# cheukwaylee/ORB_SLAM2_detailed_comments

Hardware: AMD Instinct MI355X
Metric: frames/sec ORB extract+match (1000 kp, 640x480) (higher is better)
Workload: dtype u8; 1 GPU; synthetic 640x480 mono stream, nFeatures=1000, 8 levels, scale 1.2, FAST 20/7, extract+match(t vs t-1), batch 1024 frames/GPU resident in HBM, 1 pipelines/GPU; parallelism=single GPU

## Files before the change

### include/orbx.h

```cpp
#ifndef ORBX_H
#define ORBX_H
#include <stddef.h>
#include <stdint.h>
#ifdef __cplusplus
extern "C" {
#endif

#define ORBX_ABI_VERSION 1

typedef struct orbx_keypoint {
    float x, y;
    float size;
    float angle;
    float response;
    int32_t octave;
    int32_t class_id;
} orbx_keypoint;

typedef enum orbx_status {
    ORBX_OK = 0,
    ORBX_EMPTY_IMAGE = 1,
    ORBX_BAD_ARGUMENT = 2,
    ORBX_BAD_ASPECT = 3,
    ORBX_CAPACITY = 4,
// ... 336 lines not shown
void *orbx_get_stream(orbx_handle *h);
orbx_status orbx_set_stream(orbx_handle *h, void *hip_stream);
orbx_status orbx_synchronize(orbx_handle *h);
enum {
    ORBX_K_PYR_L0 = 0, ORBX_K_PYR_RESIZE = 1, ORBX_K_FAST = 2, ORBX_K_QUADTREE = 3, ORBX_K_ORIENT = 4,
    ORBX_K_BLUR = 5, ORBX_K_DESC = 6, ORBX_K_MATCH = 7, ORBX_K_MISC = 8, ORBX_K_COUNT = 9
};
orbx_status orbx_profile_enable(orbx_handle *h, uint32_t kernel_mask);
orbx_status orbx_profile_read(orbx_handle *h, float *ms, int32_t *launches, int reset);
const char *orbx_kernel_name(int kernel_id);

orbx_status orbx_debug_candidates(orbx_handle *h, int frame, int level, orbx_keypoint *out, int cap, int *n);
orbx_status orbx_debug_level_keypoints(orbx_handle *h, int frame, int level, orbx_keypoint *out, int cap, int *n);
orbx_status orbx_debug_blur_copy(orbx_handle *h, int frame, int level, uint8_t *dst, int dst_stride);
orbx_status orbx_debug_fast_groups(orbx_handle *h, int *level0, int *total);

typedef struct orbx_pose_problem {
    int32_t frame;
    float   Tcw[16];
    const int32_t *point_index;
    int32_t npoints;
} orbx_pose_problem;
orbx_status orbx_pose_optimization_batch_device(orbx_handle *h, int nproblems, const orbx_pose_problem *problems, int npool,
                                                const float *world_pos, int nframes, const orbx_keypoint *d_keys_un,
                                                const float *d_u_right, const int32_t *d_counts, int cap, const int32_t *d_point,
                                                const float *camera4, float mbf, const float *inv_level_sigma2, int nlevels,
                                                float *d_Tcw, uint8_t *d_outlier, int32_t *d_ninliers);
orbx_status orbx_pose_optimization(orbx_handle *h, float *Tcw, int n, const orbx_keypoint *keys_un, const float *u_right,
                                   const int32_t *point, int npool, const float *world_pos, const float *camera4, float mbf,
                                   const float *inv_level_sigma2, int nlevels, uint8_t *outlier, int32_t *ninliers);
// ... 31 lines not shown
```

### orb_slam2_detailed_comments_amd/_capi.py

```python
from __future__ import annotations
import ctypes as C
import os
import numpy as np

HERE = os.path.dirname(os.path.abspath(__file__))
LIB_PATH = os.environ.get("ORBX_LIB") or os.path.join(HERE, "lib", "liborbx.so")

KP_DTYPE = np.dtype([("x", "<f4"), ("y", "<f4"), ("size", "<f4"), ("angle", "<f4"),
                     ("response", "<f4"), ("octave", "<i4"), ("class_id", "<i4")])
assert KP_DTYPE.itemsize == 28

OK, EMPTY_IMAGE, BAD_ARGUMENT, BAD_ASPECT, CAPACITY, HIP_ERROR, NO_DEVICE, UNSUPPORTED = range(8)
FP_GCC_FMA, FP_STRICT = 0, 1
PYRAMID_FORK_PADDED, PYRAMID_UPSTREAM = 0, 1
FMT_GRAY8, FMT_RGB8, FMT_BGR8, FMT_RGBA8, FMT_BGRA8 = range(5)
DEPTH_U16, DEPTH_F32 = 0, 1
K_NAMES = ("k_pyr_l0", "k_pyr_resize", "k_fast_rows", "k_quadtree", "k_orient", "k_blur", "k_describe",
           "k_match", "misc")
K_COUNT = len(K_NAMES)


class Params(C.Structure):
    _fields_ = [("nfeatures", C.c_int32), ("scale_factor", C.c_float), ("nlevels", C.c_int32),
                ("ini_th_fast", C.c_int32), ("min_th_fast", C.c_int32), ("pyramid_mode", C.c_int32),
# ... 82 lines not shown

class OrbxError(RuntimeError):
    def __init__(self, status, msg):
        super().__init__(f"orbx status {status}: {msg}")
        self.status = status


SYMBOLS = [
    "orbx_create", "orbx_destroy", "orbx_default_params", "orbx_last_error", "orbx_status_string",
    "orbx_abi_version", "orbx_get_levels", "orbx_get_scale_factor", "orbx_get_scale_tables",
    "orbx_get_features_per_level", "orbx_get_umax", "orbx_max_keypoints", "orbx_extract", "orbx_extract_batch",
    "orbx_extract_batch_device", "orbx_pyramid_level_info", "orbx_pyramid_level_device",
    "orbx_pyramid_level_copy", "orbx_match_bruteforce_device", "orbx_match_bruteforce", "orbx_hamming_matrix",
    "orbx_get_stream", "orbx_set_stream", "orbx_synchronize", "orbx_profile_enable", "orbx_profile_read",
    "orbx_kernel_name", "orbx_debug_candidates", "orbx_debug_level_keypoints", "orbx_debug_blur_copy", "orbx_debug_fast_groups",
    "orbx_grid_create", "orbx_grid_destroy", "orbx_grid_query", "orbx_three_maxima",
    "orbx_search_for_initialization", "orbx_stereo_match", "orbx_search_by_projection_frame",
    "orbx_search_by_projection_mappoints", "orbx_search_by_projection_frame_batch_device",
    "orbx_search_by_projection_mappoints_batch_device", "orbx_predict_scale_table", "orbx_predict_scale",
    "orbx_search_local_points_batch_device", "orbx_set_input_format", "orbx_search_by_bow_keyframe_frame",
    "orbx_search_by_bow_keyframes", "orbx_search_by_bow_keyframe_frame_batch", "orbx_search_by_bow_keyframes_batch", "orbx_search_for_triangulation", "orbx_triangulation_batch_create", "orbx_triangulation_batch_select", "orbx_triangulation_batch_destroy", "orbx_fuse", "orbx_fuse_sim3", "orbx_fuse_batch", "orbx_fuse_sim3_batch",
    "orbx_search_by_projection_sim3", "orbx_search_by_sim3", "orbx_search_by_projection_keyframe",
    "orbx_stereo_match_batch_device", "orbx_host_alloc", "orbx_host_free", "orbx_set_rectification", "orbx_undistort_keypoints_device",
    "orbx_grid_build_device", "orbx_gated_candidates",
    "orbx_undistort_keypoints", "orbx_image_bounds", "orbx_rgbd_depth_device", "orbx_rgbd_depth", "orbx_extract_rgbd_batch",
    "orbx_vocabulary_create", "orbx_vocabulary_destroy", "orbx_bow_transform", "orbx_bow_transform_device", "orbx_bow_vectors",
    "orbx_vocabulary_scoring", "orbx_bow_score", "orbx_kfdb_create", "orbx_kfdb_destroy", "orbx_kfdb_clear", "orbx_kfdb_size",
    "orbx_kfdb_add", "orbx_kfdb_erase", "orbx_kfdb_score_entries", "orbx_kfdb_query_reloc", "orbx_kfdb_query_loop",
    "orbx_kfdb_query_matches", "orbx_kfdb_query_touched", "orbx_kfdb_select_groups", "orbx_kfdb_state",
    "orbx_distinctive_descriptors_batch", "orbx_distinctive_descriptors_batch_device", "orbx_update_normal_and_depth_batch",
# ... 62 lines not shown
    L.orbx_sim3_batch_counts.restype = i32; L.orbx_sim3_batch_counts.argtypes = [vp, i32, vp, C.POINTER(i32)]
    L.orbx_sim3_batch_hypothesis.restype = i32; L.orbx_sim3_batch_hypothesis.argtypes = [vp, i32, i32, vp, vp]
    L.orbx_sim3_batch_destroy.restype = None; L.orbx_sim3_batch_destroy.argtypes = [vp]
    L.orbx_sim3_atan2.restype = C.c_double; L.orbx_sim3_atan2.argtypes = [C.c_double, C.c_double]
    L.orbx_get_stream.restype = vp; L.orbx_get_stream.argtypes = [vp]
    L.orbx_set_stream.restype = i32; L.orbx_set_stream.argtypes = [vp, vp]
    L.orbx_synchronize.restype = i32; L.orbx_synchronize.argtypes = [vp]
    L.orbx_profile_enable.restype = i32; L.orbx_profile_enable.argtypes = [vp, C.c_uint32]
    L.orbx_profile_read.restype = i32; L.orbx_profile_read.argtypes = [vp, vp, vp, i32]
    L.orbx_kernel_name.restype = C.c_char_p; L.orbx_kernel_name.argtypes = [i32]
    L.orbx_debug_candidates.restype = i32; L.orbx_debug_candidates.argtypes = [vp, i32, i32, vp, i32, C.POINTER(i32)]
    L.orbx_debug_level_keypoints.restype = i32
    L.orbx_debug_level_keypoints.argtypes = [vp, i32, i32, vp, i32, C.POINTER(i32)]
    L.orbx_debug_blur_copy.restype = i32; L.orbx_debug_blur_copy.argtypes = [vp, i32, i32, vp, i32]
    L.orbx_debug_fast_groups.restype = i32; L.orbx_debug_fast_groups.argtypes = [vp, C.POINTER(i32), C.POINTER(i32)]
    L.orbx_grid_create.restype = vp; L.orbx_grid_create.argtypes = [vp, i32, f32, f32, f32, f32]
    L.orbx_grid_destroy.restype = None; L.orbx_grid_destroy.argtypes = [vp]
    L.orbx_grid_query.restype = i32; L.orbx_grid_query.argtypes = [vp, f32, f32, f32, i32, i32, vp, i32]
    L.orbx_three_maxima.restype = None
    L.orbx_three_maxima.argtypes = [vp, i32, C.POINTER(i32), C.POINTER(i32), C.POINTER(i32)]
    L.orbx_search_for_initialization.restype = i32
    L.orbx_search_for_initialization.argtypes = [vp, vp, vp, i32, vp, vp, i32, vp, vp, i32, f32, i32, vp, C.POINTER(i32)]
    L.orbx_stereo_match.restype = i32
    L.orbx_stereo_match.argtypes = [vp, vp, i32, i32, vp, vp, i32, vp, vp, i32, f32, f32, vp, vp, C.POINTER(i32)]
    L.orbx_search_by_projection_frame.restype = i32
    L.orbx_search_by_projection_frame.argtypes = [vp, C.POINTER(FrameView), C.POINTER(LastFrameView), f32, i32, i32, vp,
                                                  C.POINTER(i32)]
    L.orbx_search_by_projection_mappoints.restype = i32
    L.orbx_search_by_projection_mappoints.argtypes = [vp, C.POINTER(FrameView), vp, C.POINTER(MapPointView), f32, f32, vp,
                                                      C.POINTER(i32)]
# ... 120 lines not shown
```

### orb_slam2_detailed_comments_amd/csrc/orbx_kernels.hip

```cpp
#include "orbx_device.h"
#include "orbx_inplace.h"
#include "orbx_fast_net.h"
#include "orbx_track.h"
#include "../../include/orbx_pattern_data.h"

#define L0_ROWS 8
#ifndef L0_FF
#define L0_FF 1
#endif
#ifndef RR_FF
#define RR_FF 1
#endif
#define QT_KPT ORBX_QT_KPT
#ifndef QT_DROP_STAGE_A
#define QT_DROP_STAGE_A 1
#endif
#ifndef QT_ONE_SCAN
#define QT_ONE_SCAN 1
#endif
#ifndef QT_REG_SIZE
#define QT_REG_SIZE 1
#endif
#ifndef QT_CENSUS_NODES
#define QT_CENSUS_NODES 1
// ... 1543 lines not shown
                s0 = s0 + (float)r3 * k3;
                o = (int)__builtin_rintf(s0);
            } else {
                o = (55 * r0 + 49 * r1 + 34 * r2 + 18 * r3 + (1 << 15)) >> 16;
            }
            o = min(max(o, 0), 255);
            outv |= (uint32_t)o << (8 * i);
        }
        *(uint32_t *)(out + (long long)Y * L.pitch + X) = outv;
    }
}

__constant__ int4 c_pattern_lane[64];
__constant__ uint32_t c_orient_w[64][12];
__constant__ uint32_t c_blur_b[3][64][4];

#ifndef DS_ORDER
#define DS_ORDER 1
#endif
#define DS_R 21
#define DS_W (2 * DS_R + 1)
#define DS_PP 44
#define DS_HC 40
#ifndef DS_COLFIRST
#define DS_COLFIRST 1
#endif
#ifndef DS_ALIAS
#define DS_ALIAS 1
#endif
#ifndef DS_MFMA
#define DS_MFMA 1
#endif
#define DS_VC 44
#define DS_VR 40
#ifndef DS_WPB
#define DS_WPB 1
#endif
#ifndef DS_WPS
#define DS_WPS 7
#endif
typedef const __attribute__((address_space(3))) uint16_t *orbx_lds_u16p;
typedef const __attribute__((address_space(3))) uint32_t *orbx_lds_u32p;
__device__ __forceinline__ uint32_t orbx_ds_tap(uint32_t adr) {
    typedef unsigned short u16x2 __attribute__((ext_vector_type(2)));
    const bool odd = (adr & 2u) != 0;
    const orbx_lds_u32p wp = (orbx_lds_u32p)(uintptr_t)(adr & ~3u);
    const uint32_t d0 = wp[0], d1 = wp[1], d2 = wp[2], d3 = wp[3];
    const uint32_t w0 = odd ? (18u << 16) : (18u | (34u << 16)), w1 = odd ? (34u | (49u << 16)) : (49u | (55u << 16)),
                   w2 = odd ? (55u | (49u << 16)) : (49u | (34u << 16)), w3 = odd ? (34u | (18u << 16)) : 18u;
    uint32_t I = __builtin_amdgcn_udot2(__builtin_bit_cast(u16x2, d0), __builtin_bit_cast(u16x2, w0), 0u, false);
    I = __builtin_amdgcn_udot2(__builtin_bit_cast(u16x2, d1), __builtin_bit_cast(u16x2, w1), I, false);
    I = __builtin_amdgcn_udot2(__builtin_bit_cast(u16x2, d2), __builtin_bit_cast(u16x2, w2), I, false);
    I = __builtin_amdgcn_udot2(__builtin_bit_cast(u16x2, d3), __builtin_bit_cast(u16x2, w3), I, false);
    return I;
}
template <int FPM, bool INPLACE>
__global__ __launch_bounds__(64 * DS_WPB, DS_WPS) void k_describe(DGeom g, const uint8_t *__restrict__ pyr,
                                                  const uint32_t *__restrict__ lvl_kp,
                                                  const int *__restrict__ lvl_count,
                                                  float *__restrict__ lvl_angle, orbx_keypoint *__restrict__ kps,
                                                  uint8_t *__restrict__ desc, int *__restrict__ counts,
                                                  int *__restrict__ status, int cap, int dbg_stop, int nframes, OrbxRaw0 raw) {
#ifndef ORBX_TIMING_KNOBS
    dbg_stop = 0;
#endif
#if DS_COLFIRST && DS_ALIAS
    __shared__ __attribute__((aligned(16))) uint16_t s_h[DS_WPB][DS_VR * DS_VC];
#else
    __shared__ uint32_t s_patch[DS_WPB][DS_W * DS_PP / 4 + 4];
    __shared__ __attribute__((aligned(16))) uint16_t s_h[DS_WPB][DS_COLFIRST ? DS_VR * DS_VC : DS_W * DS_HC];
#endif
    const int lane = threadIdx.x & 63, wv_id = __builtin_amdgcn_readfirstlane(threadIdx.x >> 6);
#if DS_ORDER == 1
    const int f = blockIdx.y * 8 + (blockIdx.x & 7);
    const int oi = (blockIdx.x >> 3) * DS_WPB + wv_id;
    if (f >= nframes) return;
#else
    const int f = blockIdx.x;
    const int oi = blockIdx.y * DS_WPB + wv_id;
#endif
    const int *lc = lvl_count + f * g.nlevels;
    int total = 0, level = 0, slot = oi;
#ifndef DS_LEVELS8
#define DS_LEVELS8 1
#endif
    if (DS_LEVELS8 && g.nlevels == 8) {
        const int4 ca = *(const int4 *)lc, cb = *(const int4 *)(lc + 4);
        const int cnt[8] = {ca.x, ca.y, ca.z, ca.w, cb.x, cb.y, cb.z, cb.w};
        int base = 0;
#pragma unroll
        for (int l = 0; l < 8; ++l) {
            if (oi >= total) { level = l; base = total; }
            total += cnt[l];
        }
        slot = g.lv[level].kp_begin + (oi - base);
    } else {
#pragma unroll
    for (int l = 0; l < ORBX_MAX_LEVELS; ++l) {
        if (l < g.nlevels) {
            if (oi >= total) { level = l; slot = g.lv[l].kp_begin + (oi - total); }
            total += lc[l];
        }
    }
    }
    if (oi == 0 && lane == 0) {
        counts[f] = min(total, cap);
        if (total > cap) atomicMax(&status[f], (int)ORBX_CAPACITY);
    }
    if (oi >= min(total, cap) || dbg_stop == 4) return;
#if DS_COLFIRST && DS_ALIAS
    uint32_t *patch = (uint32_t *)s_h[wv_id];
#else
    uint32_t *patch = s_patch[wv_id];
#endif
    uint16_t *hrow = s_h[wv_id];
    const uint32_t pos = lvl_kp[(long long)f * g.kp_total + slot];
    const int4 pat = c_pattern_lane[lane];
    const DLevel &L = g.lv[level];
    const int x = (int)(pos & 0xfff) + (ORBX_EDGE - 3), y = (int)((pos >> 12) & 0xfff) + (ORBX_EDGE - 3);
    const bool ip0 = INPLACE && level == 0;
    const uint8_t *img = ip0 ? raw.img + (long long)f * raw.frame_stride : pyr + (long long)f * g.pyr_bytes + L.off;
    const int spitch = ip0 ? raw.stride : L.pitch;
    const int px0 = x - DS_R + (ip0 ? -ORBX_EDGE : L.org), py0 = y - DS_R + (ip0 ? -ORBX_EDGE : L.org);
    const int xa = px0 & ~3;
    const bool interior = ip0 ? orbx_ip_desc_interior(px0, py0, raw.W, raw.H)
                              : px0 >= 0 && py0 >= 0 && xa + 48 <= L.pitch && px0 + 2 * DS_R < L.pw && py0 + 2 * DS_R < L.ph;
    {
        if (interior) {
            const int dq = lane & 3, rq = lane >> 2;
            const uint32_t shift = (uint32_t)(px0 & 3);
            const uint8_t *p0 = img + (__mul24(py0, spitch) + xa + 12 * dq);
            orbx_uint3_u tv[3];
#pragma unroll
            for (int k = 0; k < 3; ++k) tv[k] = *(const orbx_uint3_u *)(p0 + __mul24(min(16 * k + rq, DS_W - 1), spitch));
#pragma unroll
            for (int k = 0; k < 3; ++k) {
                const uint32_t nxt = orbx_lane_above(tv[k].x);
                const int r = 16 * k + rq;
                if (r < DS_W) {
                    uint32_t *d = patch + r * (DS_PP / 4) + 3 * dq;
                    d[0] = __builtin_amdgcn_alignbyte(tv[k].y, tv[k].x, shift);
                    d[1] = __builtin_amdgcn_alignbyte(tv[k].z, tv[k].y, shift);
                    if (dq < 3) d[2] = __builtin_amdgcn_alignbyte(nxt, tv[k].z, shift);
                }
            }
        } else if (ip0) {
            const int dq = lane & 3, rq = lane >> 2;
            const int ws = orbx_ip_desc_ws(px0, raw.W);
            const int e = px0 - ws;
            const uint32_t shift = (uint32_t)(e & 3);
            const int dd = e >> 2;
            orbx_uint3_u tv[3];
#pragma unroll
            for (int k = 0; k < 3; ++k)
                tv[k] = *(const orbx_uint3_u *)(img + orbx_ip_row_off(orbx_ip_map(py0 + ORBX_EDGE + min(16 * k + rq, DS_W - 1), raw.H), raw.stride, ws + 12 * dq));
#pragma unroll
            for (int k = 0; k < 3; ++k) {
                const uint32_t nxt = orbx_lane_above(tv[k].x);
                const int r = 16 * k + rq;
                if (r < DS_W) {
                    uint32_t *d = patch + r * (DS_PP / 4);
                    const int D = 3 * dq - dd;
                    const uint32_t f0 = __builtin_amdgcn_alignbyte(tv[k].y, tv[k].x, shift), f1 = __builtin_amdgcn_alignbyte(tv[k].z, tv[k].y, shift),
                                   f2 = __builtin_amdgcn_alignbyte(nxt, tv[k].z, shift);
                    if (D >= 0 && D < DS_PP / 4) d[D] = f0;
                    if (D + 1 >= 0 && D + 1 < DS_PP / 4) d[D + 1] = f1;
                    if (D + 2 >= 0 && D + 2 < DS_PP / 4) d[D + 2] = f2;
                    if (dq == 0 && D - 1 >= 0 && D - 1 < DS_PP / 4) d[D - 1] = __builtin_amdgcn_alignbyte(tv[k].x, 0u, shift);
                }
            }
            const int c_end_l = px0 < 0 ? min(-px0, DS_W) : 0, c_beg_r = max(raw.W - px0, 0);
            if (c_end_l > 0 || c_beg_r < DS_W) {
                orbx_wave_sync();
                uint8_t *pb = (uint8_t *)patch + min(lane, DS_W - 1) * DS_PP;
                const uint8_t *grow = img + orbx_ip_row_off(orbx_ip_map(py0 + ORBX_EDGE + min(lane, DS_W - 1), raw.H), raw.stride, 0);
                for (int c = 0; c < DS_W; ++c) {
                    if (c >= c_end_l && c < c_beg_r) { c = c_beg_r - 1; continue; }
                    const int j = orbx_ip_map(px0 + ORBX_EDGE + c, raw.W);
                    const int sp = j - px0;
                    const uint8_t v = (sp >= 0 && sp < DS_PP) ? pb[sp] : grow[j];
                    if (lane < DS_W) pb[c] = v;
                }
            }
        } else {
            uint8_t *pb = (uint8_t *)patch;
            for (int i = lane; i < DS_W * DS_W; i += 64) {
                const int r = i / DS_W, c = i - r * DS_W;
                const int sy = orbx_reflect101(py0 + r, L.ph), sx = orbx_reflect101(px0 + c, L.pw);
                pb[r * DS_PP + c] = img[(long long)sy * L.pitch + sx];
            }
        }
        orbx_wave_sync();
        if (dbg_stop == 1) return;
        float angle_deg;
        {
            const int row = lane >> 1, half = lane & 1;
            const uint32_t *pr = patch + min(row + (DS_R - ORBX_HALF_PATCH), DS_W - 1) * (DS_PP / 4) + 1 + 5 * half;
            const uint4 wa = *(const uint4 *)&c_orient_w[lane][0], wb = *(const uint4 *)&c_orient_w[lane][4], wc = *(const uint4 *)&c_orient_w[lane][8];
            const uint32_t p0 = pr[0], p1 = pr[1], p2 = pr[2], p3 = pr[3], p4 = pr[4];
            uint32_t A = __builtin_amdgcn_udot4(p0, wa.x, 0u, false), S = __builtin_amdgcn_udot4(p0, wb.y, 0u, false);
            A = __builtin_amdgcn_udot4(p1, wa.y, A, false); S = __builtin_amdgcn_udot4(p1, wb.z, S, false);
            A = __builtin_amdgcn_udot4(p2, wa.z, A, false); S = __builtin_amdgcn_udot4(p2, wb.w, S, false);
            A = __builtin_amdgcn_udot4(p3, wa.w, A, false); S = __builtin_amdgcn_udot4(p3, wc.x, S, false);
            A = __builtin_amdgcn_udot4(p4, wb.x, A, false); S = __builtin_amdgcn_udot4(p4, wc.y, S, false);
            int m10 = (int)A - 16 * (int)S;
            int m01 = __mul24(row - ORBX_HALF_PATCH, (int)S);
            m10 = orbx_wave_sum(m10);
            m01 = orbx_wave_sum(m01);
            angle_deg = orbx_fast_atan2((float)m01, (float)m10);
            if (lane == 0) lvl_angle[(long long)f * g.kp_total + slot] = angle_deg;
        }
        if (dbg_stop == 2) return;
#if DS_COLFIRST && DS_MFMA
        {
            typedef int i32x4 __attribute__((ext_vector_type(4)));
            const int m = lane & 15, gq = lane >> 4;
            i32x4 A[3], Bm[3];
#pragma unroll
            for (int t = 0; t < 3; ++t) {
                const uint32_t *ap = patch + (16 * t + m) * (DS_PP / 4) + 4 * gq;
                A[t][0] = (int)(ap[0] ^ 0x80808080u); A[t][1] = (int)(ap[1] ^ 0x80808080u);
                A[t][2] = (int)(ap[2] ^ 0x80808080u); A[t][3] = (int)(ap[3] ^ 0x80808080u);
            }
#pragma unroll
            for (int j = 0; j < 3; ++j) {
                const uint4 b4 = *(const uint4 *)&c_blur_b[j][lane][0];
                Bm[j][0] = (int)b4.x; Bm[j][1] = (int)b4.y; Bm[j][2] = (int)b4.z; Bm[j][3] = (int)b4.w;
            }
            const i32x4 c0 = {128 * 257, 128 * 257, 128 * 257, 128 * 257};
            uint32_t *vo = (uint32_t *)hrow + m * (DS_VC / 2) + 2 * gq;
#pragma unroll
            for (int j = 0; j < 3; ++j) {
#pragma unroll
                for (int t = 0; t < 3; ++t) {
                    const i32x4 acc = __builtin_amdgcn_mfma_i32_16x16x64_i8(A[t], Bm[j], c0, 0, 0, 0);
                    if ((j < 2 || m < DS_W - 6 - 32) && (t < 2 || gq < 3))
                        *(uint2 *)(vo + (16 * j) * (DS_VC / 2) + 8 * t) =
                            make_uint2((uint32_t)acc[0] | ((uint32_t)acc[1] << 16), (uint32_t)acc[2] | ((uint32_t)acc[3] << 16));
                }
            }
        }
#elif DS_COLFIRST
        {
            typedef unsigned short u16x2 __attribute__((ext_vector_type(2)));
            const int seg = (lane * 373) >> 12, cg = lane - 11 * seg;
            if (seg < 5) {
                uint32_t pa[14], pb[14];
#pragma unroll
                for (int j = 0; j < 14; ++j) {
                    const uint32_t d = patch[min(8 * seg + j, DS_W - 1) * (DS_PP / 4) + cg];
                    pa[j] = __builtin_amdgcn_perm(0u, d, 0x0c010c00u);
                    pb[j] = __builtin_amdgcn_perm(0u, d, 0x0c030c02u);
                }
// ... 29 lines not shown
            o.y = hv[2] | (hv[3] << 16);
            o.z = hv[4] | (hv[5] << 16);
            o.w = hv[6] | (hv[7] << 16);
            *(uint4 *)(hrow + r * DS_HC + 8 * q8) = o;
        }
#endif
        __builtin_amdgcn_fence(__ATOMIC_RELEASE, "wavefront");
        __builtin_amdgcn_wave_barrier();
        __builtin_amdgcn_fence(__ATOMIC_ACQUIRE, "wavefront");
        if (dbg_stop == 3) return;
        const float factorPI = (float)(3.1415926535897932384626433832795 / 180.f);
        const float angle = angle_deg * factorPI;
                const OrbxSinCos sc = orbx_sincosf_pinned(angle);
        const float a = sc.c, b = sc.s;
        const int wvec = (L.pw - 2 * L.org) & ~3;
        const int pw4[4] = {pat.x, pat.y, pat.z, pat.w};
        unsigned long long words[4];
        if (x + (DS_R - 3) < wvec) {
#if DS_COLFIRST
            const uint32_t cbias = (uint32_t)(2 * ((DS_R - 3) * DS_VC + (DS_R - 3))) - 0x400000u * (2u * DS_VC) - (0x4B400000u << 1);
#else
            const uint32_t cbias = (uint32_t)(2 * ((DS_R - 3) * DS_HC + (DS_R - 3))) - 0x400000u * (2u * DS_HC) - (0x4B400000u << 1);
#endif
            const uint32_t hbase = (uint32_t)(uintptr_t)(orbx_lds_u16p)hrow + cbias;
            float tv[8];
            float nb = -b;
            asm("" : "+v"(nb));
#pragma unroll
            for (int r = 0; r < 4; ++r) {
#pragma unroll
                for (int s2 = 0; s2 < 2; ++s2) {
                    const float px = (float)(signed char)((pw4[r] >> (16 * s2)) & 0xff);
                    const float py = (float)(signed char)((pw4[r] >> (16 * s2 + 8)) & 0xff);
                    float fy, fx;
                    if (FPM == ORBX_FP_GCC_FMA) {
                        fy = __builtin_fmaf(px, b, py * a);
                        fx = __builtin_fmaf(px, a, py * nb);
                    } else {
                        fy = px * b + py * a;
                        fx = px * a + py * nb;
                    }
                    const uint32_t uy = __float_as_uint(fy + 12582912.0f), ux = __float_as_uint(fx + 12582912.0f);
#if DS_COLFIRST
#if DS_MFMA
                    uint32_t ay = (uy << 1) + hbase;
                    asm("" : "+v"(ay));
                    const uint32_t adr = __umul24(ux, 2u * DS_VC) + ay;
#else
                    const uint32_t adr = __umul24(uy, 2u * DS_VC) + ((ux << 1) + hbase);
#endif
                    const uint32_t I = orbx_ds_tap(adr);
#else
                    uint32_t adr = __umul24(uy, 2u * DS_HC) + ((ux << 1) + hbase);
                    asm("" : "+v"(adr));
                    const orbx_lds_u16p hp = (orbx_lds_u16p)(uintptr_t)adr;
                    const uint32_t r0 = hp[3 * DS_HC], r1 = (uint32_t)hp[2 * DS_HC] + hp[4 * DS_HC],
                                   r2 = (uint32_t)hp[1 * DS_HC] + hp[5 * DS_HC], r3 = (uint32_t)hp[0] + hp[6 * DS_HC];
                    const uint32_t I = __umul24(55u, r0) + __umul24(49u, r1) + __umul24(34u, r2) + __umul24(18u, r3);
#endif
                    tv[2 * r + s2] = __builtin_fminf(__builtin_rintf((float)I * (1.f / 65536.f)), 255.f);
                }
            }
#pragma unroll
            for (int r = 0; r < 4; ++r) words[r] = orbx_ballot(tv[2 * r] < tv[2 * r + 1]);
        } else {
            int tval[8];
#pragma unroll
            for (int r = 0; r < 4; ++r) {
#pragma unroll
                for (int s2 = 0; s2 < 2; ++s2) {
                    const float px = (float)(signed char)((pw4[r] >> (16 * s2)) & 0xff);
                    const float py = (float)(signed char)((pw4[r] >> (16 * s2 + 8)) & 0xff);
                    float fy, fx;
                    if (FPM == ORBX_FP_GCC_FMA) {
                        fy = __builtin_fmaf(px, b, py * a);
                        fx = __builtin_fmaf(px, a, -(py * b));
                    } else {
                        fy = px * b + py * a;
                        fx = px * a - py * b;
                    }
                    const int iy = (int)__builtin_rintf(fy), ix = (int)__builtin_rintf(fx);
#if DS_COLFIRST
#if DS_MFMA
                    const uint32_t I = orbx_ds_tap((uint32_t)(uintptr_t)(orbx_lds_u16p)hrow + 2u * (uint32_t)(__mul24(ix + DS_R - 3, DS_VC) + (iy + DS_R - 3)));
#else
                    const uint32_t I = orbx_ds_tap((uint32_t)(uintptr_t)(orbx_lds_u16p)hrow + 2u * (uint32_t)(__mul24(iy + DS_R - 3, DS_VC) + (ix + DS_R - 3)));
#endif
#else
                    const uint16_t *hp = hrow + __mul24(iy + DS_R - 3, DS_HC) + (ix + DS_R - 3);
                    const uint32_t r0 = hp[3 * DS_HC], r1 = (uint32_t)hp[2 * DS_HC] + hp[4 * DS_HC],
                                   r2 = (uint32_t)hp[1 * DS_HC] + hp[5 * DS_HC], r3 = (uint32_t)hp[0] + hp[6 * DS_HC];
                    const uint32_t I = __umul24(55u, r0) + __umul24(49u, r1) + __umul24(34u, r2) + __umul24(18u, r3);
#endif
                    const uint32_t tie = x + ix >= wvec ? 1u : ((I >> 16) & 1u);
                    tval[2 * r + s2] = (int)min((I + 0x7fffu + tie) >> 16, 255u);
                }
            }
#pragma unroll
            for (int r = 0; r < 4; ++r) words[r] = orbx_ballot(tval[2 * r] < tval[2 * r + 1]);
        }
        if (lane < 4) {
            unsigned long long w = lane == 0 ? words[0] : lane == 1 ? words[1] : lane == 2 ? words[2] : words[3];
            *(unsigned long long *)(desc + ((long long)f * cap + oi) * 32 + 8 * lane) = w;
        }
        if (lane == 0) {
            orbx_keypoint kp;
            float fx = (float)x, fy = (float)y;
            if (level != 0) { fx = fx * L.scale; fy = fy * L.scale; }
            kp.x = fx; kp.y = fy;
            kp.size = L.size;
// ... 1835 lines not shown
            const bool in = i < len && orbx_sim3_inlier(T12, T21, K1, K2, v, v + 3, v + 8, v + 10, v[6], v[7]);
            const unsigned long long word = orbx_ballot(in);
            if (lane == 0) mw[(base + sub) >> 6] = word;
            cnt += __popcll(word);
        }
    }
    if (active && lane == 0) A.counts[D.iter_off + it] = cnt;
}

#include "orbx_launch.h"
#include <string>
#include <cstdio>
#include <cstring>
#include <mutex>

hipError_t orbx_upload_pattern() {
    signed char t[64 * 16];
    for (int l = 0; l < 64; ++l)
        for (int r = 0; r < 4; ++r)
            for (int k = 0; k < 4; ++k) t[l * 16 + r * 4 + k] = ORBX_PATTERN_I8[(r * 64 + l) * 4 + k];
    hipError_t e = hipMemcpyToSymbol(HIP_SYMBOL(c_pattern_lane), t, sizeof(t));
    if (e != hipSuccess) return e;
    orbx_params p;
    orbx_default_params(&p);
    OrbxTables tab;
    orbx_build_tables(p, tab);
    static uint32_t w[64][12];
    memset(w, 0, sizeof(w));
    for (int lane = 0; lane < 62; ++lane) {
        const int row = lane >> 1, half = lane & 1, v = row - ORBX_HALF_PATCH;
        const int d = tab.umax[v < 0 ? -v : v];
        for (int k = 0; k < 5; ++k)
            for (int b = 0; b < 4; ++b) {
                const int col = 4 * (1 + 5 * half + k) + b;
                const int u = col - DS_R;
                if (col < DS_W && u >= -d && u <= d) {
// ... 384 lines not shown
```

### orb_slam2_detailed_comments_amd/csrc/orbx_launch.h

```cpp
#pragma once
#include <hip/hip_runtime.h>
#include "orbx_device.h"
#include "orbx_inplace.h"
#include "orbx_track.h"
#include "orbx_mappoint.h"
#include "orbx_pose.h"
#include "orbx_sim3.h"

hipError_t orbx_upload_pattern();
size_t orbx_quadtree_smem(int ncap, int lds_keys);
hipError_t orbx_quadtree_prepare(size_t smem);
void orbx_launch_clear(hipStream_t s, int *a, int na, int *b, int nb, int *c, int nc);
void orbx_launch_pyr_l0(hipStream_t s, const DGeom &g, int B, const uint8_t *imgs, int W, int H, int stride,
                        long long frame_stride, uint8_t *pyr, int *status, int *cand_cursor);
void orbx_launch_pyr_l0_color(hipStream_t s, const DGeom &g, int B, const uint8_t *imgs, int W, int H, int stride,
                              long long frame_stride, uint8_t *pyr, int nch, int r_off, int b_off, int *status, int *cand_cursor);
void orbx_launch_pyr_l0_remap(hipStream_t s, const DGeom &g, int B, const uint8_t *imgs, int W, int H, int stride,
                              long long frame_stride, uint8_t *pyr, const uint2 *rect, int *status, int *cand_cursor);
void orbx_launch_pyr_resize(hipStream_t s, const DGeom &g, int B, int level, const OrbxTap *taps, uint8_t *pyr, bool narrow,
                            int rpw_forced = 0);
void orbx_launch_fast_rows(hipStream_t s, const DGeom &g, int B, const OrbxCell *cells, const OrbxFastGroup *groups,
                           int ngroups, const uint8_t *pyr, uint2 *cand, int *cand_cursor, int *status, int max_ch, int lcap,
                           int dbg_stop, int lds_floor = 0, const OrbxRaw0 *raw = nullptr, bool l0_only = false);
void orbx_launch_pyr_resize_l1(hipStream_t s, const DGeom &g, int B, const OrbxTap *taps_l1, const OrbxRaw0 &raw, uint8_t *pyr,
// ... 78 lines not shown
```

### orb_slam2_detailed_comments_amd/csrc/orbx_pyramid.cpp

```cpp
#include <cstring>
#include <algorithm>
#include <utility>
#include <vector>
#include "orbx_handle.h"

static inline size_t level_view_off(const OrbxLevelGeom &L) { return (size_t)L.off + (size_t)L.org * L.pitch + L.org; }
static orbx_status check_level(orbx_handle *h, int frame, int level) {
    if (!h) return orbx_fail(ORBX_BAD_ARGUMENT, "null handle");
    if (!h->configured || h->last_batch == 0) return orbx_fail(ORBX_BAD_ARGUMENT, "no frame extracted yet");
    if (level < 0 || level >= h->p.nlevels || frame < 0 || frame >= h->last_batch) return orbx_fail(ORBX_BAD_ARGUMENT, "frame/level out of range");
    return ORBX_OK;
}
extern "C" orbx_status orbx_pyramid_level_info(orbx_handle *h, int level, int *width, int *height, int *pitch) {
    orbx_status st = check_level(h, 0, level);
    if (st != ORBX_OK) return st;
    if (width) *width = h->geom.lv[level].vw;
    if (height) *height = h->geom.lv[level].vh;
    if (pitch) *pitch = h->geom.lv[level].pitch;
    return ORBX_OK;
}
static orbx_status ensure_level0(orbx_handle *h) {
    if (!h->l0_pending) return ORBX_OK;
    HIPCHK(hipSetDevice(h->dev));
    { ProfScope ps(h, ORBX_K_PYR_L0);
// ... 92 lines not shown
    }
    for (int i = 0; i < cnt && i < cap; ++i) {
        orbx_keypoint k;
        k.x = (float)((pos[i] & 0xfff) + ORBX_EDGE - 3); k.y = (float)(((pos[i] >> 12) & 0xfff) + ORBX_EDGE - 3);
        k.size = L.size; k.angle = ang[i]; k.response = (float)(pos[i] >> 24); k.octave = level; k.class_id = -1;
        out[i] = k;
    }
    if (cnt > cap) return orbx_fail(ORBX_CAPACITY, "output capacity");
    return ORBX_OK;
}

extern "C" orbx_status orbx_debug_fast_groups(orbx_handle *h, int *level0, int *total) {
    if (!h || !h->configured) return orbx_fail(ORBX_BAD_ARGUMENT, "no batch has been extracted on this handle");
    if (level0) *level0 = h->l0_groups;
    if (total) *total = (int)h->geom.fast_groups.size();
    return ORBX_OK;
}

static OrbxStereoGeom stereo_geom(const orbx_handle *hl, float mb, float mbf) {
    OrbxStereoGeom sg;
    memset(&sg, 0, sizeof(sg));
    sg.nlevels = hl->p.nlevels; sg.nrows0 = hl->geom.lv[0].vh; sg.mb = mb; sg.mbf = mbf;
    for (int l = 0; l < sg.nlevels; ++l) {
        const OrbxLevelGeom &L = hl->geom.lv[l];
        sg.scale[l] = hl->tab.scale[l]; sg.inv_scale[l] = hl->tab.inv_scale[l];
        sg.pw[l] = L.vw; sg.ph[l] = L.vh; sg.pitch[l] = L.pitch;
        sg.off[l] = (long long)level_view_off(L);
    }
    return sg;
}
// ... 117 lines not shown
```

Measured before the change: 402,200 frames/s.

## Restructure describe kernel: slot-indexed level lookup, early table loads, perm packing

The describe kernel now maps each wave directly to a per-level keypoint slot, holding the level bases and counts in scalar registers, instead of walking cumulative counts from a compacted index. Constant-table loads (pattern, orientation weights, blur MFMA operands) are hoisted ahead of the patch staging behind a scheduling barrier so their latency overlaps the patch loads. MFMA output packing uses byte-permute instructions. Optional batched LDS taps and a float pattern table are added behind macros that default off. The aim is to cut address arithmetic and latency stalls, at the cost of more scalar and vector registers and possibly launching waves that exit early on empty slots.

```diff
diff --git a/include/orbx.h b/include/orbx.h
--- a/include/orbx.h
+++ b/include/orbx.h
@@ -374,6 +374,7 @@
 orbx_status orbx_debug_level_keypoints(orbx_handle *h, int frame, int level, orbx_keypoint *out, int cap, int *n);
 orbx_status orbx_debug_blur_copy(orbx_handle *h, int frame, int level, uint8_t *dst, int dst_stride);
 orbx_status orbx_debug_fast_groups(orbx_handle *h, int *level0, int *total);
+orbx_status orbx_debug_describe_pattern(int8_t *lane_i8_1024, float *lane_f32_1024);
 
 typedef struct orbx_pose_problem {
     int32_t frame;
diff --git a/orb_slam2_detailed_comments_amd/_capi.py b/orb_slam2_detailed_comments_amd/_capi.py
--- a/orb_slam2_detailed_comments_amd/_capi.py
+++ b/orb_slam2_detailed_comments_amd/_capi.py
@@ -120,6 +120,7 @@
     "orbx_pyramid_level_copy", "orbx_match_bruteforce_device", "orbx_match_bruteforce", "orbx_hamming_matrix",
     "orbx_get_stream", "orbx_set_stream", "orbx_synchronize", "orbx_profile_enable", "orbx_profile_read",
     "orbx_kernel_name", "orbx_debug_candidates", "orbx_debug_level_keypoints", "orbx_debug_blur_copy", "orbx_debug_fast_groups",
+    "orbx_debug_describe_pattern",
     "orbx_grid_create", "orbx_grid_destroy", "orbx_grid_query", "orbx_three_maxima",
     "orbx_search_for_initialization", "orbx_stereo_match", "orbx_search_by_projection_frame",
     "orbx_search_by_projection_mappoints", "orbx_search_by_projection_frame_batch_device",
@@ -212,6 +213,8 @@
     L.orbx_debug_level_keypoints.argtypes = [vp, i32, i32, vp, i32, C.POINTER(i32)]
     L.orbx_debug_blur_copy.restype = i32; L.orbx_debug_blur_copy.argtypes = [vp, i32, i32, vp, i32]
     L.orbx_debug_fast_groups.restype = i32; L.orbx_debug_fast_groups.argtypes = [vp, C.POINTER(i32), C.POINTER(i32)]
+    if hasattr(L, "orbx_debug_describe_pattern"):
+        L.orbx_debug_describe_pattern.restype = i32; L.orbx_debug_describe_pattern.argtypes = [vp, vp]
     L.orbx_grid_create.restype = vp; L.orbx_grid_create.argtypes = [vp, i32, f32, f32, f32, f32]
     L.orbx_grid_destroy.restype = None; L.orbx_grid_destroy.argtypes = [vp]
     L.orbx_grid_query.restype = i32; L.orbx_grid_query.argtypes = [vp, f32, f32, f32, i32, i32, vp, i32]
diff --git a/orb_slam2_detailed_comments_amd/csrc/orbx_kernels.hip b/orb_slam2_detailed_comments_amd/csrc/orbx_kernels.hip
--- a/orb_slam2_detailed_comments_amd/csrc/orbx_kernels.hip
+++ b/orb_slam2_detailed_comments_amd/csrc/orbx_kernels.hip
@@ -1581,6 +1581,7 @@
 __constant__ int4 c_pattern_lane[64];
 __constant__ uint32_t c_orient_w[64][12];
 __constant__ uint32_t c_blur_b[3][64][4];
+__constant__ float4 c_pattern_f32[64][4];
 
 #ifndef DS_ORDER
 #define DS_ORDER 1
@@ -1606,20 +1607,46 @@
 #ifndef DS_WPS
 #define DS_WPS 7
 #endif
+#ifndef DS_SLOT
+#define DS_SLOT 1
+#endif
+#ifndef DS_EARLY_TABLES
+#define DS_EARLY_TABLES 7
+#endif
+#ifndef DS_TAP_BATCH
+#define DS_TAP_BATCH 1
+#endif
+#ifndef DS_PATTERN_F32
+#define DS_PATTERN_F32 0
+#endif
+#ifndef DS_PACK_PERM
+#define DS_PACK_PERM 1
+#endif
 typedef const __attribute__((address_space(3))) uint16_t *orbx_lds_u16p;
 typedef const __attribute__((address_space(3))) uint32_t *orbx_lds_u32p;
-__device__ __forceinline__ uint32_t orbx_ds_tap(uint32_t adr) {
+template <int N>
+__device__ __forceinline__ void orbx_ds_taps(const uint32_t (&adr)[N], uint32_t (&I)[N]) {
     typedef unsigned short u16x2 __attribute__((ext_vector_type(2)));
-    const bool odd = (adr & 2u) != 0;
-    const orbx_lds_u32p wp = (orbx_lds_u32p)(uintptr_t)(adr & ~3u);
-    const uint32_t d0 = wp[0], d1 = wp[1], d2 = wp[2], d3 = wp[3];
-    const uint32_t w0 = odd ? (18u << 16) : (18u | (34u << 16)), w1 = odd ? (34u | (49u << 16)) : (49u | (55u << 16)),
-                   w2 = odd ? (55u | (49u << 16)) : (49u | (34u << 16)), w3 = odd ? (34u | (18u << 16)) : 18u;
-    uint32_t I = __builtin_amdgcn_udot2(__builtin_bit_cast(u16x2, d0), __builtin_bit_cast(u16x2, w0), 0u, false);
-    I = __builtin_amdgcn_udot2(__builtin_bit_cast(u16x2, d1), __builtin_bit_cast(u16x2, w1), I, false);
-    I = __builtin_amdgcn_udot2(__builtin_bit_cast(u16x2, d2), __builtin_bit_cast(u16x2, w2), I, false);
-    I = __builtin_amdgcn_udot2(__builtin_bit_cast(u16x2, d3), __builtin_bit_cast(u16x2, w3), I, false);
-    return I;
+    uint32_t d[N][4];
+#pragma unroll
+    for (int k = 0; k < N; ++k) {
+        const orbx_lds_u32p wp = (orbx_lds_u32p)(uintptr_t)(adr[k] & ~3u);
+        d[k][0] = wp[0]; d[k][1] = wp[1]; d[k][2] = wp[2]; d[k][3] = wp[3];
+    }
+    uint32_t w[N][4];
+#pragma unroll
+    for (int k = 0; k < N; ++k) {
+        const bool odd = (adr[k] & 2u) != 0;
+        w[k][0] = odd ? (18u << 16) : (18u | (34u << 16)); w[k][1] = odd ? (34u | (49u << 16)) : (49u | (55u << 16));
+        w[k][2] = odd ? (55u | (49u << 16)) : (49u | (34u << 16)); w[k][3] = odd ? (34u | (18u << 16)) : 18u;
+    }
+#pragma unroll
+    for (int k = 0; k < N; ++k) I[k] = 0u;
+#pragma unroll
+    for (int i = 0; i < 4; ++i)
+#pragma unroll
+        for (int k = 0; k < N; ++k)
+            I[k] = __builtin_amdgcn_udot2(__builtin_bit_cast(u16x2, d[k][i]), __builtin_bit_cast(u16x2, w[k][i]), I[k], false);
 }
 template <int FPM, bool INPLACE>
 __global__ __launch_bounds__(64 * DS_WPB, DS_WPS) void k_describe(DGeom g, const uint8_t *__restrict__ pyr,
@@ -1638,19 +1665,75 @@
     __shared__ __attribute__((aligned(16))) uint16_t s_h[DS_WPB][DS_COLFIRST ? DS_VR * DS_VC : DS_W * DS_HC];
 #endif
     const int lane = threadIdx.x & 63, wv_id = __builtin_amdgcn_readfirstlane(threadIdx.x >> 6);
+#if DS_SLOT
+    int kbv[8];
+#pragma unroll
+    for (int l = 0; l < 8; ++l) kbv[l] = g.lv[l].kp_begin;
+    asm("" : "+s"(nframes), "+s"(cap), "+s"(kbv[0]), "+s"(kbv[1]), "+s"(kbv[2]), "+s"(kbv[3]), "+s"(kbv[4]), "+s"(kbv[5]), "+s"(kbv[6]), "+s"(kbv[7])
+           : "s"(g.nlevels), "s"(g.kp_total), "s"(g.pyr_bytes), "s"(lvl_kp), "s"(lvl_count), "s"(pyr));
+#endif
 #if DS_ORDER == 1
     const int f = blockIdx.y * 8 + (blockIdx.x & 7);
-    const int oi = (blockIdx.x >> 3) * DS_WPB + wv_id;
+    const int wi = (blockIdx.x >> 3) * DS_WPB + wv_id;
     if (f >= nframes) return;
 #else
     const int f = blockIdx.x;
-    const int oi = blockIdx.y * DS_WPB + wv_id;
+    const int wi = blockIdx.y * DS_WPB + wv_id;
 #endif
     const int *lc = lvl_count + f * g.nlevels;
-    int total = 0, level = 0, slot = oi;
+    int total = 0, level = 0;
 #ifndef DS_LEVELS8
 #define DS_LEVELS8 1
 #endif
+#if DS_SLOT
+    const int slot = wi;
+    if (DS_WPB > 1 && slot >= g.kp_total) return;
+    const bool all8 = DS_LEVELS8 && g.nlevels == 8;
+    int kb = kbv[0];
+    if (all8) {
+#pragma unroll
+        for (int l = 1; l < 8; ++l)
+            if (slot >= kbv[l]) { level = l; kb = kbv[l]; }
+    } else {
+#pragma unroll
+        for (int l = 1; l < ORBX_MAX_LEVELS; ++l)
+            if (l < g.nlevels && slot >= g.lv[l].kp_begin) { level = l; kb = g.lv[l].kp_begin; }
+    }
+    uint32_t pos = lvl_kp[(long long)f * g.kp_total + slot];
+    struct { int pw, ph, pitch, org; long long off; float scale, size; } L =
+        {g.lv[level].pw, g.lv[level].ph, g.lv[level].pitch, g.lv[level].org, g.lv[level].off, g.lv[level].scale, g.lv[level].size};
+    int base = 0, mine = 0;
+    if (all8) {
+        int4 ca = *(const int4 *)lc, cb = *(const int4 *)(lc + 4);
+        asm("" : "+s"(pos), "+s"(L.pw), "+s"(L.ph), "+s"(L.pitch), "+s"(L.org), "+s"(L.off), "+s"(L.scale), "+s"(L.size),
+                 "+s"(ca.x), "+s"(ca.y), "+s"(ca.z), "+s"(ca.w), "+s"(cb.x), "+s"(cb.y), "+s"(cb.z), "+s"(cb.w));
+        const int cnt[8] = {ca.x, ca.y, ca.z, ca.w, cb.x, cb.y, cb.z, cb.w};
+#pragma unroll
+        for (int l = 0; l < 8; ++l) {
+            if (l < level) base += cnt[l];
+            if (l == level) mine = cnt[l];
+            total += cnt[l];
+        }
+    } else {
+#pragma unroll
+        for (int l = 0; l < ORBX_MAX_LEVELS; ++l) {
+            if (l < g.nlevels) {
+                const int c = lc[l];
+                if (l < level) base += c;
+                if (l == level) mine = c;
+                total += c;
+            }
+        }
+    }
+    const int oi = base + (slot - kb);
+    if (slot == 0 && lane == 0) {
+        counts[f] = min(total, cap);
+        if (total > cap) atomicMax(&status[f], (int)ORBX_CAPACITY);
+    }
+    if (slot - kb >= mine || oi >= min(total, cap) || dbg_stop == 4) return;
+#else
+    const int oi = wi;
+    int slot = oi;
     if (DS_LEVELS8 && g.nlevels == 8) {
         const int4 ca = *(const int4 *)lc, cb = *(const int4 *)(lc + 4);
         const int cnt[8] = {ca.x, ca.y, ca.z, ca.w, cb.x, cb.y, cb.z, cb.w};
@@ -1675,15 +1758,32 @@
         if (total > cap) atomicMax(&status[f], (int)ORBX_CAPACITY);
     }
     if (oi >= min(total, cap) || dbg_stop == 4) return;
+    const uint32_t pos = lvl_kp[(long long)f * g.kp_total + slot];
+    const DLevel &L = g.lv[level];
+#endif
 #if DS_COLFIRST && DS_ALIAS
     uint32_t *patch = (uint32_t *)s_h[wv_id];
 #else
     uint32_t *patch = s_patch[wv_id];
 #endif
     uint16_t *hrow = s_h[wv_id];
-    const uint32_t pos = lvl_kp[(long long)f * g.kp_total + slot];
-    const int4 pat = c_pattern_lane[lane];
-    const DLevel &L = g.lv[level];
+#if DS_PATTERN_F32
+    float4 patf[4];
+#define DS_LOAD_PATTERN() do { _Pragma("unroll") for (int r = 0; r < 4; ++r) patf[r] = c_pattern_f32[lane][r]; } while (0)
+#else
+    int4 pat;
+#define DS_LOAD_PATTERN() do { pat = c_pattern_lane[lane]; } while (0)
+#endif
+    uint4 wa, wb, wc;
+#define DS_LOAD_ORIENT_W() do { wa = *(const uint4 *)&c_orient_w[lane][0]; wb = *(const uint4 *)&c_orient_w[lane][4]; wc = *(const uint4 *)&c_orient_w[lane][8]; } while (0)
+#if DS_COLFIRST && DS_MFMA
+    uint4 b4[3];
+#define DS_LOAD_BLUR_B() do { _Pragma("unroll") for (int j = 0; j < 3; ++j) b4[j] = *(const uint4 *)&c_blur_b[j][lane][0]; } while (0)
+#else
+#define DS_LOAD_BLUR_B() do { } while (0)
+#endif
+#define DS_LOAD_EARLY() do { if (DS_EARLY_TABLES) __builtin_amdgcn_sched_barrier(0); if (DS_EARLY_TABLES & 1) DS_LOAD_PATTERN(); if (DS_EARLY_TABLES & 2) DS_LOAD_ORIENT_W(); if (DS_EARLY_TABLES & 4) DS_LOAD_BLUR_B(); } while (0)
+    if (!(DS_EARLY_TABLES & 1)) DS_LOAD_PATTERN();
     const int x = (int)(pos & 0xfff) + (ORBX_EDGE - 3), y = (int)((pos >> 12) & 0xfff) + (ORBX_EDGE - 3);
     const bool ip0 = INPLACE && level == 0;
     const uint8_t *img = ip0 ? raw.img + (long long)f * raw.frame_stride : pyr + (long long)f * g.pyr_bytes + L.off;
@@ -1700,6 +1800,7 @@
             orbx_uint3_u tv[3];
 #pragma unroll
             for (int k = 0; k < 3; ++k) tv[k] = *(const orbx_uint3_u *)(p0 + __mul24(min(16 * k + rq, DS_W - 1), spitch));
+            DS_LOAD_EARLY();
 #pragma unroll
             for (int k = 0; k < 3; ++k) {
                 const uint32_t nxt = orbx_lane_above(tv[k].x);
@@ -1721,6 +1822,7 @@
 #pragma unroll
             for (int k = 0; k < 3; ++k)
                 tv[k] = *(const orbx_uint3_u *)(img + orbx_ip_row_off(orbx_ip_map(py0 + ORBX_EDGE + min(16 * k + rq, DS_W - 1), raw.H), raw.stride, ws + 12 * dq));
+            DS_LOAD_EARLY();
 #pragma unroll
             for (int k = 0; k < 3; ++k) {
                 const uint32_t nxt = orbx_lane_above(tv[k].x);
@@ -1751,6 +1853,7 @@
             }
         } else {
             uint8_t *pb = (uint8_t *)patch;
+            DS_LOAD_EARLY();
             for (int i = lane; i < DS_W * DS_W; i += 64) {
                 const int r = i / DS_W, c = i - r * DS_W;
                 const int sy = orbx_reflect101(py0 + r, L.ph), sx = orbx_reflect101(px0 + c, L.pw);
@@ -1763,7 +1866,7 @@
         {
             const int row = lane >> 1, half = lane & 1;
             const uint32_t *pr = patch + min(row + (DS_R - ORBX_HALF_PATCH), DS_W - 1) * (DS_PP / 4) + 1 + 5 * half;
-            const uint4 wa = *(const uint4 *)&c_orient_w[lane][0], wb = *(const uint4 *)&c_orient_w[lane][4], wc = *(const uint4 *)&c_orient_w[lane][8];
+            if (!(DS_EARLY_TABLES & 2)) DS_LOAD_ORIENT_W();
             const uint32_t p0 = pr[0], p1 = pr[1], p2 = pr[2], p3 = pr[3], p4 = pr[4];
             uint32_t A = __builtin_amdgcn_udot4(p0, wa.x, 0u, false), S = __builtin_amdgcn_udot4(p0, wb.y, 0u, false);
             A = __builtin_amdgcn_udot4(p1, wa.y, A, false); S = __builtin_amdgcn_udot4(p1, wb.z, S, false);
@@ -1789,10 +1892,10 @@
                 A[t][0] = (int)(ap[0] ^ 0x80808080u); A[t][1] = (int)(ap[1] ^ 0x80808080u);
                 A[t][2] = (int)(ap[2] ^ 0x80808080u); A[t][3] = (int)(ap[3] ^ 0x80808080u);
             }
+            if (!(DS_EARLY_TABLES & 4)) DS_LOAD_BLUR_B();
 #pragma unroll
             for (int j = 0; j < 3; ++j) {
-                const uint4 b4 = *(const uint4 *)&c_blur_b[j][lane][0];
-                Bm[j][0] = (int)b4.x; Bm[j][1] = (int)b4.y; Bm[j][2] = (int)b4.z; Bm[j][3] = (int)b4.w;
+                Bm[j][0] = (int)b4[j].x; Bm[j][1] = (int)b4[j].y; Bm[j][2] = (int)b4[j].z; Bm[j][3] = (int)b4[j].w;
             }
             const i32x4 c0 = {128 * 257, 128 * 257, 128 * 257, 128 * 257};
             uint32_t *vo = (uint32_t *)hrow + m * (DS_VC / 2) + 2 * gq;
@@ -1802,8 +1905,14 @@
                 for (int t = 0; t < 3; ++t) {
                     const i32x4 acc = __builtin_amdgcn_mfma_i32_16x16x64_i8(A[t], Bm[j], c0, 0, 0, 0);
                     if ((j < 2 || m < DS_W - 6 - 32) && (t < 2 || gq < 3))
+#if DS_PACK_PERM
+                        *(uint2 *)(vo + (16 * j) * (DS_VC / 2) + 8 * t) =
+                            make_uint2(__builtin_amdgcn_perm((uint32_t)acc[1], (uint32_t)acc[0], 0x05040100u),
+                                       __builtin_amdgcn_perm((uint32_t)acc[3], (uint32_t)acc[2], 0x05040100u));
+#else
                         *(uint2 *)(vo + (16 * j) * (DS_VC / 2) + 8 * t) =
                             make_uint2((uint32_t)acc[0] | ((uint32_t)acc[1] << 16), (uint32_t)acc[2] | ((uint32_t)acc[3] << 16));
+#endif
                 }
             }
         }
@@ -1863,7 +1972,14 @@
                 const OrbxSinCos sc = orbx_sincosf_pinned(angle);
         const float a = sc.c, b = sc.s;
         const int wvec = (L.pw - 2 * L.org) & ~3;
+#if DS_PATTERN_F32
+#define DS_PX(t) (((t) & 1) ? patf[(t) >> 1].z : patf[(t) >> 1].x)
+#define DS_PY(t) (((t) & 1) ? patf[(t) >> 1].w : patf[(t) >> 1].y)
+#else
         const int pw4[4] = {pat.x, pat.y, pat.z, pat.w};
+#define DS_PX(t) ((float)(signed char)((pw4[(t) >> 1] >> (16 * ((t) & 1))) & 0xff))
+#define DS_PY(t) ((float)(signed char)((pw4[(t) >> 1] >> (16 * ((t) & 1) + 8)) & 0xff))
+#endif
         unsigned long long words[4];
         if (x + (DS_R - 3) < wvec) {
 #if DS_COLFIRST
@@ -1876,11 +1992,11 @@
             float nb = -b;
             asm("" : "+v"(nb));
 #pragma unroll
-            for (int r = 0; r < 4; ++r) {
-#pragma unroll
-                for (int s2 = 0; s2 < 2; ++s2) {
-                    const float px = (float)(signed char)((pw4[r] >> (16 * s2)) & 0xff);
-                    const float py = (float)(signed char)((pw4[r] >> (16 * s2 + 8)) & 0xff);
+            for (int t0 = 0; t0 < 8; t0 += DS_TAP_BATCH) {
+                uint32_t adr[DS_TAP_BATCH], I[DS_TAP_BATCH];
+#pragma unroll
+                for (int k = 0; k < DS_TAP_BATCH; ++k) {
+                    const float px = DS_PX(t0 + k), py = DS_PY(t0 + k);
                     float fy, fx;
                     if (FPM == ORBX_FP_GCC_FMA) {
                         fy = __builtin_fmaf(px, b, py * a);
@@ -1894,32 +2010,40 @@
 #if DS_MFMA
                     uint32_t ay = (uy << 1) + hbase;
                     asm("" : "+v"(ay));
-                    const uint32_t adr = __umul24(ux, 2u * DS_VC) + ay;
+                    adr[k] = __umul24(ux, 2u * DS_VC) + ay;
 #else
-                    const uint32_t adr = __umul24(uy, 2u * DS_VC) + ((ux << 1) + hbase);
-#endif
-                    const uint32_t I = orbx_ds_tap(adr);
+                    adr[k] = __umul24(uy, 2u * DS_VC) + ((ux << 1) + hbase);
+#endif
 #else
-                    uint32_t adr = __umul24(uy, 2u * DS_HC) + ((ux << 1) + hbase);
-                    asm("" : "+v"(adr));
-                    const orbx_lds_u16p hp = (orbx_lds_u16p)(uintptr_t)adr;
+                    adr[k] = __umul24(uy, 2u * DS_HC) + ((ux << 1) + hbase);
+                    asm("" : "+v"(adr[k]));
+#endif
+                }
+#if DS_COLFIRST
+                orbx_ds_taps<DS_TAP_BATCH>(adr, I);
+#else
+#pragma unroll
+                for (int k = 0; k < DS_TAP_BATCH; ++k) {
+                    const orbx_lds_u16p hp = (orbx_lds_u16p)(uintptr_t)adr[k];
                     const uint32_t r0 = hp[3 * DS_HC], r1 = (uint32_t)hp[2 * DS_HC] + hp[4 * DS_HC],
                                    r2 = (uint32_t)hp[1 * DS_HC] + hp[5 * DS_HC], r3 = (uint32_t)hp[0] + hp[6 * DS_HC];
-                    const uint32_t I = __umul24(55u, r0) + __umul24(49u, r1) + __umul24(34u, r2) + __umul24(18u, r3);
-#endif
-                    tv[2 * r + s2] = __builtin_fminf(__builtin_rintf((float)I * (1.f / 65536.f)), 255.f);
+                    I[k] = __umul24(55u, r0) + __umul24(49u, r1) + __umul24(34u, r2) + __umul24(18u, r3);
                 }
+#endif
+#pragma unroll
+                for (int k = 0; k < DS_TAP_BATCH; ++k) tv[t0 + k] = __builtin_fminf(__builtin_rintf((float)I[k] * (1.f / 65536.f)), 255.f);
             }
 #pragma unroll
             for (int r = 0; r < 4; ++r) words[r] = orbx_ballot(tv[2 * r] < tv[2 * r + 1]);
         } else {
             int tval[8];
 #pragma unroll
-            for (int r = 0; r < 4; ++r) {
-#pragma unroll
-                for (int s2 = 0; s2 < 2; ++s2) {
-                    const float px = (float)(signed char)((pw4[r] >> (16 * s2)) & 0xff);
-                    const float py = (float)(signed char)((pw4[r] >> (16 * s2 + 8)) & 0xff);
+            for (int t0 = 0; t0 < 8; t0 += DS_TAP_BATCH) {
+                uint32_t adr[DS_TAP_BATCH], I[DS_TAP_BATCH];
+                int ixs[DS_TAP_BATCH];
+#pragma unroll
+                for (int k = 0; k < DS_TAP_BATCH; ++k) {
+                    const float px = DS_PX(t0 + k), py = DS_PY(t0 + k);
                     float fy, fx;
                     if (FPM == ORBX_FP_GCC_FMA) {
                         fy = __builtin_fmaf(px, b, py * a);
@@ -1929,20 +2053,32 @@
                         fx = px * a - py * b;
                     }
                     const int iy = (int)__builtin_rintf(fy), ix = (int)__builtin_rintf(fx);
+                    ixs[k] = ix;
 #if DS_COLFIRST
 #if DS_MFMA
-                    const uint32_t I = orbx_ds_tap((uint32_t)(uintptr_t)(orbx_lds_u16p)hrow + 2u * (uint32_t)(__mul24(ix + DS_R - 3, DS_VC) + (iy + DS_R - 3)));
+                    adr[k] = (uint32_t)(uintptr_t)(orbx_lds_u16p)hrow + 2u * (uint32_t)(__mul24(ix + DS_R - 3, DS_VC) + (iy + DS_R - 3));
 #else
-                    const uint32_t I = orbx_ds_tap((uint32_t)(uintptr_t)(orbx_lds_u16p)hrow + 2u * (uint32_t)(__mul24(iy + DS_R - 3, DS_VC) + (ix + DS_R - 3)));
+                    adr[k] = (uint32_t)(uintptr_t)(orbx_lds_u16p)hrow + 2u * (uint32_t)(__mul24(iy + DS_R - 3, DS_VC) + (ix + DS_R - 3));
 #endif
 #else
-                    const uint16_t *hp = hrow + __mul24(iy + DS_R - 3, DS_HC) + (ix + DS_R - 3);
+                    adr[k] = (uint32_t)(__mul24(iy + DS_R - 3, DS_HC) + (ix + DS_R - 3));
+#endif
+                }
+#if DS_COLFIRST
+                orbx_ds_taps<DS_TAP_BATCH>(adr, I);
+#else
+#pragma unroll
+                for (int k = 0; k < DS_TAP_BATCH; ++k) {
+                    const uint16_t *hp = hrow + adr[k];
                     const uint32_t r0 = hp[3 * DS_HC], r1 = (uint32_t)hp[2 * DS_HC] + hp[4 * DS_HC],
                                    r2 = (uint32_t)hp[1 * DS_HC] + hp[5 * DS_HC], r3 = (uint32_t)hp[0] + hp[6 * DS_HC];
-                    const uint32_t I = __umul24(55u, r0) + __umul24(49u, r1) + __umul24(34u, r2) + __umul24(18u, r3);
-#endif
-                    const uint32_t tie = x + ix >= wvec ? 1u : ((I >> 16) & 1u);
-                    tval[2 * r + s2] = (int)min((I + 0x7fffu + tie) >> 16, 255u);
+                    I[k] = __umul24(55u, r0) + __umul24(49u, r1) + __umul24(34u, r2) + __umul24(18u, r3);
+                }
+#endif
+#pragma unroll
+                for (int k = 0; k < DS_TAP_BATCH; ++k) {
+                    const uint32_t tie = x + ixs[k] >= wvec ? 1u : ((I[k] >> 16) & 1u);
+                    tval[t0 + k] = (int)min((I[k] + 0x7fffu + tie) >> 16, 255u);
                 }
             }
 #pragma unroll
@@ -3808,12 +3944,19 @@
 #include <cstring>
 #include <mutex>
 
+void orbx_pattern_lane_tables(signed char *i8, float *f32) {
+    for (int l = 0; l < 64; ++l)
+        for (int r = 0; r < 4; ++r)
+            for (int k = 0; k < 4; ++k) i8[l * 16 + r * 4 + k] = ORBX_PATTERN_I8[(r * 64 + l) * 4 + k];
+    for (int i = 0; i < 64 * 16; ++i) f32[i] = (float)i8[i];
+}
 hipError_t orbx_upload_pattern() {
     signed char t[64 * 16];
-    for (int l = 0; l < 64; ++l)
-        for (int r = 0; r < 4; ++r)
-            for (int k = 0; k < 4; ++k) t[l * 16 + r * 4 + k] = ORBX_PATTERN_I8[(r * 64 + l) * 4 + k];
+    static float tf[64 * 16];
+    orbx_pattern_lane_tables(t, tf);
     hipError_t e = hipMemcpyToSymbol(HIP_SYMBOL(c_pattern_lane), t, sizeof(t));
+    if (e != hipSuccess) return e;
+    e = hipMemcpyToSymbol(HIP_SYMBOL(c_pattern_f32), tf, sizeof(tf));
     if (e != hipSuccess) return e;
     orbx_params p;
     orbx_default_params(&p);
diff --git a/orb_slam2_detailed_comments_amd/csrc/orbx_launch.h b/orb_slam2_detailed_comments_amd/csrc/orbx_launch.h
--- a/orb_slam2_detailed_comments_amd/csrc/orbx_launch.h
+++ b/orb_slam2_detailed_comments_amd/csrc/orbx_launch.h
@@ -8,6 +8,7 @@
 #include "orbx_sim3.h"
 
 hipError_t orbx_upload_pattern();
+void orbx_pattern_lane_tables(signed char *i8, float *f32);
 size_t orbx_quadtree_smem(int ncap, int lds_keys);
 hipError_t orbx_quadtree_prepare(size_t smem);
 void orbx_launch_clear(hipStream_t s, int *a, int na, int *b, int nb, int *c, int nc);
diff --git a/orb_slam2_detailed_comments_amd/csrc/orbx_pyramid.cpp b/orb_slam2_detailed_comments_amd/csrc/orbx_pyramid.cpp
--- a/orb_slam2_detailed_comments_amd/csrc/orbx_pyramid.cpp
+++ b/orb_slam2_detailed_comments_amd/csrc/orbx_pyramid.cpp
@@ -130,6 +130,11 @@
     if (!h || !h->configured) return orbx_fail(ORBX_BAD_ARGUMENT, "no batch has been extracted on this handle");
     if (level0) *level0 = h->l0_groups;
     if (total) *total = (int)h->geom.fast_groups.size();
+    return ORBX_OK;
+}
+extern "C" orbx_status orbx_debug_describe_pattern(int8_t *lane_i8_1024, float *lane_f32_1024) {
+    if (!lane_i8_1024 || !lane_f32_1024) return orbx_fail(ORBX_BAD_ARGUMENT, "null table");
+    orbx_pattern_lane_tables((signed char *)lane_i8_1024, lane_f32_1024);
     return ORBX_OK;
 }
 
```

Result: faster. 408,100 frames/s (median of 6 runs) (+1.5%).
